# sjulier/Refactored_ORB_SLAM2

Hardware: AMD Instinct MI355X
Metric: frames/s (extract+match) at KITTI 1241×376, 2000 feat; 1/2/4/8 GPU + CPU ref (higher is better)
Workload: dtype u8; 1 GPU; kitti_stereo_1241x376_2000feat_8lvl: 2x ORBextractor + ComputeStereoMatches + SearchByProjection(cur,last); parallelism=frame-shard x1, collective=none, driver=torch, queries=one pass: orbfe_track_queries_stereo_device

## Files before the change

refactored_orb_slam2_amd/csrc/extract_kernels.hip:

```cpp
#include <stdlib.h>
#include <string.h>

#include "orbfe_internal.h"
#include "../../include/orb_pattern_data.h"

#define WAVE 64

__device__ __forceinline__ int wave_incl_scan(int v) {
  v += __builtin_amdgcn_update_dpp(0, v, 0x111, 0xf, 0xf, false);
  v += __builtin_amdgcn_update_dpp(0, v, 0x112, 0xf, 0xf, false);
  v += __builtin_amdgcn_update_dpp(0, v, 0x114, 0xf, 0xf, false);
  v += __builtin_amdgcn_update_dpp(0, v, 0x118, 0xf, 0xf, false);
  v += __builtin_amdgcn_update_dpp(0, v, 0x142, 0xa, 0xf, false);
  v += __builtin_amdgcn_update_dpp(0, v, 0x143, 0xc, 0xf, false);
  return v;
}

template <int T>
__device__ __forceinline__ int block_incl_scan_t(int v, int* tmp, int* total) {
  const int tid = threadIdx.x;
  const int lane = tid & (WAVE - 1), wid = tid >> 6;
  int s = wave_incl_scan(v);
  if (T == WAVE) {
    *total = __builtin_amdgcn_readlane(s, WAVE - 1);
// ... 377 lines not shown
#if FC_TIMING
__device__ unsigned long long g_fc_prof[4096 * 8];
#define FC_T(i) do { const uint32_t _t = (uint32_t)__builtin_readcyclecounter(); tacc##i += _t - tprev; tprev = _t; } while (0)
extern "C" int orbfe_debug_fc_profile(unsigned long long* out, int reset) {
  static unsigned long long h[4096 * 8];
  if (hipMemcpyFromSymbol(h, HIP_SYMBOL(g_fc_prof), sizeof(h)) != hipSuccess) return 1;
  for (int i = 0; i < 8; i++) out[i] = 0;
  for (int sl = 0; sl < 4096; sl++)
    for (int i = 0; i < 8; i++) out[i] += h[sl * 8 + i];
  if (reset) { memset(h, 0, sizeof(h)); if (hipMemcpyToSymbol(HIP_SYMBOL(g_fc_prof), h, sizeof(h)) != hipSuccess) return 1; }
  return 0;
}
#else
#define FC_T(i)
#endif
#ifndef FC_SCALAR_CELL
#define FC_SCALAR_CELL 1
#endif
#ifndef FC_PE_COND
#define FC_PE_COND 1
#endif
#ifndef FC_WAVES_PER_EU
#define FC_WAVES_PER_EU 7
#endif
#ifndef FC_WG_WAVES
#define FC_WG_WAVES 4
#endif
__host__ __device__ inline int fc_wave_lds(int rows_max, int pb, int sc_bytes, int nbw) {
  return rows_max * pb + sc_bytes + nbw * 4 + FC_LIST_CAP * 2 + (FC_T2_QUEUE ? FC_Q1_CAP * 2 : 0) + FC_LDS_PAD;
}
template <int PB, int NLD>
__global__ __launch_bounds__(64 * FC_WG_WAVES, FC_WAVES_PER_EU) void fast_cells_kernel(PyrView pyr, const CellDesc* __restrict__ cells,
                                                          const FastGroup* __restrict__ runs, int n_runs, int total_cells,
                                                          int rows_max, int sc_bytes, int nbw, int32_t* __restrict__ cell_cnt,
                                                          uint32_t* __restrict__ slots, unsigned long long slots_per_image,
                                                          int ini_th, int min_th, int xcd_run_shift) {
  extern __shared__ __attribute__((aligned(16))) uint8_t fc_smem[];
  const int lane = threadIdx.x & (WAVE - 1), wid = __builtin_amdgcn_readfirstlane((int)(threadIdx.x >> 6));
  uint8_t* tile = fc_smem + wid * fc_wave_lds(rows_max, PB, sc_bytes, nbw);
  uint8_t* sc = tile + rows_max * PB;
  uint32_t* scb = reinterpret_cast<uint32_t*>(sc + sc_bytes);
  uint16_t* list = reinterpret_cast<uint16_t*>(scb + nbw);
#if FC_T2_QUEUE
  uint16_t* q1 = list + FC_LIST_CAP;
#endif
  int img = blockIdx.y;
  const int nblk = (n_runs + FC_WG_WAVES - 1) / FC_WG_WAVES;
  const int q = blockIdx.x >> 3;
  const int unit = 8 << (xcd_run_shift < 0 ? 0 : xcd_run_shift);
  int bid = (xcd_run_shift < 0 || (int)blockIdx.x >= (nblk / unit) * unit)
                ? (int)blockIdx.x
                : ((q >> xcd_run_shift) << (xcd_run_shift + 3)) + ((blockIdx.x & 7) << xcd_run_shift) +
                      (q & ((1 << xcd_run_shift) - 1));
  if (xcd_run_shift == -2) {
    const unsigned gx = gridDim.x;
    const unsigned lin = blockIdx.y * gx + blockIdx.x;
    const unsigned grp = lin / (8u * gx);
    if (8u * grp + 8u <= gridDim.y) {
      const unsigned within = lin - grp * 8u * gx;
      img = (int)(8u * grp + (within & 7u));
      bid = (int)(within >> 3);
    }
  }
  const int rid = bid * FC_WG_WAVES + wid;
  if (rid >= n_runs) return;
  const FastGroup g = runs[rid];
  const int level = g.level;
  const int pitch = pyr.pitch[level];
  const uint8_t* plane = pyr.base[level] + (size_t)img * pyr.img_stride[level];
  const uint32_t tile_a = (uint32_t)(uintptr_t)tile;

#if FC_TIMING
  uint32_t tacc0 = 0, tacc1 = 0, tacc2 = 0, tacc3 = 0, tacc4 = 0, tacc5 = 0, tprev = (uint32_t)__builtin_readcyclecounter();
#endif
  static_assert(sizeof(CellDesc) == 32, "eight dwords");
  auto load_cell = [&](int idx) {
    const __attribute__((address_space(4))) uint32_t* q =
        (const __attribute__((address_space(4))) uint32_t*)(uintptr_t)(cells + __builtin_amdgcn_readfirstlane(idx));
    CellDesc c;
    uint32_t w[8];
#pragma unroll
    for (int j = 0; j < 8; j++) w[j] = q[j];
    __builtin_memcpy(&c, w, sizeof(c));
    return c;
  };
  for (int k = 0; k < g.n_cells; k++) {
    const CellDesc cd = FC_SCALAR_CELL ? load_cell(g.first_cell + k) : cells[g.first_cell + k];
    uint4 pv[NLD];
    uint32_t pe[NLD];
    {
      const int ndq = ((cd.x0 & 15) + (((cd.x0 & 15) + 3) & 1) + cd.cols + 15) >> 4;
      const uint8_t* src = plane + (size_t)cd.y0 * pitch + (cd.x0 & ~15);
      const bool ltiled = (pyr.tiled >> level) & 1u;
      const uint32_t tstep = (uint32_t)(pitch >> 4) << 7;
      auto chunk_ptr = [&](int r, int c) {
        const int y = cd.y0 + r;
        return ltiled ? plane + (uint32_t)(y >> 3) * tstep + ((uint32_t)(((cd.x0 & ~15) >> 4) + c) << 7) + (uint32_t)((y & 7) * 16)
                      : src + (size_t)r * pitch + 16 * c;
      };
      auto front_ptr = [&](int r, int c, const uint8_t* p) {
        return ltiled ? p - 128 + 12 : p - 4;
      };
      if constexpr (PB == 64) {
        const int c = min(lane & 3, ndq - 1);
#pragma unroll
        for (int kk = 0; kk < NLD; kk++) {
          const int r = min((lane >> 2) + 16 * kk, cd.rows - 1);
          const uint8_t* p = chunk_ptr(r, c);          pv[kk] = *reinterpret_cast<const uint4*>(p);
#if FC_PE_COND
          pe[kk] = ((cd.x0 & 15) + 3) & 1 ? *reinterpret_cast<const uint32_t*>(front_ptr(r, c, p)) : 0u;
#else
          pe[kk] = *reinterpret_cast<const uint32_t*>(front_ptr(r, c, p));
#endif
        }
      } else {
        const int items = cd.rows * ndq;
        const float inv = 1.0f / (float)ndq;
#pragma unroll
        for (int kk = 0; kk < NLD; kk++) {
          const int i = min(lane + WAVE * kk, items - 1);
          const int r = (int)((i + 0.5f) * inv), c = i - r * ndq;
          const uint8_t* p = chunk_ptr(r, c);
          pv[kk] = *reinterpret_cast<const uint4*>(p);
          pe[kk] = *reinterpret_cast<const uint32_t*>(front_ptr(r, c, p));
        }
      }
    }
#if FC_TIMING
    asm volatile("s_waitcnt vmcnt(0)" ::: "memory");
    FC_T(0);
#endif
    const int cols = cd.cols, rows = cd.rows;
    const int xo = cd.x0 & 15, sh = (xo + 3) & 1, xs = xo + sh;
    const int ndq = (xs + cols + 15) >> 4;
    const int th = rows - 6, tw = cols - 6;
    const int c_lo = xs + 3, c_hi = xs + cols - 3;
    const int SCP = tw + 2;
    const int bsh = tw > 32 ? 6 : 5;
    {
      const int items = rows * ndq;
      const float inv = 1.0f / (float)ndq;
#pragma unroll
      for (int kk = 0; kk < NLD; kk++) {
        int r, c;
        if constexpr (PB == 64) { r = min((lane >> 2) + 16 * kk, rows - 1); c = min(lane & 3, ndq - 1); }
        else { const int i = min(lane + WAVE * kk, items - 1); r = (int)((i + 0.5f) * inv); c = i - r * ndq; }
        uint4 d = pv[kk];
        if (sh) {
          d.w = __builtin_amdgcn_alignbyte(d.w, d.z, 3);
          d.z = __builtin_amdgcn_alignbyte(d.z, d.y, 3);
          d.y = __builtin_amdgcn_alignbyte(d.y, d.x, 3);
          d.x = __builtin_amdgcn_alignbyte(d.x, pe[kk], 3);
        }
        *reinterpret_cast<uint4*>(tile + r * PB + 16 * c) = d;
      }
      const int nsc = ((th + 2) * SCP + 15) >> 4;
      for (int i = lane; i < nsc; i += WAVE) reinterpret_cast<uint4*>(sc)[i] = make_uint4(0, 0, 0, 0);
    }
    FC_T(1);

    auto score_list = [&](int n, bool mark, int th_cur) {
      int n_end = n;
      for (int done = 0; done < n_end;) {
        const int start = done;
        const int lim = min(start + WAVE, n_end);
        const int i = start + lane;
        done = lim;
        uint32_t en = i < lim ? list[i] : 0u;
        int e = (int)(en & 0x3fffu);
        int y = PB == 64 ? (e >> 6) : (int)((e + 0.5f) * (1.0f / PB));
        int x = e - y * PB;
// ... 44 lines not shown
            atomicOr(&scb[p >> 5], 1u << (p & 31));
          }
        }
      }
    };

    uint32_t keep[2] = {0u, 0u};
    int total = 0;
    bool was_flushed = false;
    for (int pass = 0; pass < 2; pass++) {
      const int th_cur = pass ? min_th : ini_th;
      const uint32_t C = (uint32_t)(0x8000 - th_cur - 1) * 0x00010001u;
      bool flushed = false;
      int wcnt = 0;
      if (th > 0 && tw > 0) {
        const int ppr = cd.ppr;
        const int RI = cd.ri;
        const int rl = (int)((lane + 0.5f) * cd.inv_ppr), pl = lane - rl * ppr;
        const bool lane_ok = rl < RI;
        const int n_it = cd.n_it;
        const int x = c_lo + 2 * pl;
        const bool odd2 = (x & 2) != 0;
        const uint32_t selV = odd2 ? 0x0c030c02u : 0x0c010c00u;
#if !FC_T2_QUEUE
        const uint32_t selX = odd2 ? 0x0c010c00u : 0x0c030c02u;
#endif
        const uint32_t selM = odd2 ? 0x0c040c03u : 0x0c020c01u;
        const uint32_t selP = odd2 ? 0x0c020c01u : 0x0c040c03u;
        uint32_t a0 = tile_a + rl * PB + ((x >> 2) << 2) - 4;
        uint32_t a1 = a0 + (odd2 ? 4u : 0u);
#if !(FC_T2_QUEUE && FC_T1_ASM)
        const uint32_t ec = (uint32_t)(3 * PB + 4 + (x & 3)) - tile_a;
        int rows_left = lane_ok ? th - rl : 0;
#endif
#if FC_T2_QUEUE && FC_T1_ASM
        const unsigned long long m_full = __ballot(lane_ok), m_last = __ballot(lane_ok && rl < th - (n_it - 1) * RI);
        const uint32_t oddbit = odd2 ? 1u : 0u;
        const uint32_t q_base = (uint32_t)(uintptr_t)q1, q_limit = q_base + 2u * WAVE;
        uint32_t q_addr = q_base;
        int it = 0;
        for (int phase = 0; phase < 2; phase++) {
          const unsigned long long actm = phase ? m_last : m_full;
          const int nit = __builtin_amdgcn_readfirstlane(phase ? n_it : n_it - 1);
          const int step = __builtin_amdgcn_readfirstlane(RI * PB);
          for (;;) {
            if (it < nit) {
              uint32_t tV, tA, tB, tC, tD, tE;
              uint32_t sc_;
              asm volatile(
                  "1:\n\t"
                  "ds_read2_b32 v[64:65], %[a0] offset0:1 offset1:%[K61]\n\t"
                  "ds_read2_b32 v[66:67], %[a0] offset0:%[K30] offset1:%[K31]\n\t"
                  "ds_read2_b32 v[68:69], %[a1] offset0:%[K31] offset1:%[K32]\n\t"
                  "s_add_u32 %[it], %[it], 1\n\t"
                  "s_waitcnt lgkmcnt(0)\n\t"
                  "v_perm_b32 %[tV], 0, v67, %[selV]\n\t"
                  "v_perm_b32 %[tA], 0, v64, %[selV]\n\t"
                  "v_perm_b32 %[tB], 0, v65, %[selV]\n\t"
                  "v_perm_b32 %[tC], v67, v66, %[selM]\n\t"
// ... 111 lines not shown
            const uint32_t D0 = (uint32_t)(pc >> 32), Dm = (uint32_t)pc;
            const uint32_t V = __builtin_amdgcn_perm(0u, D0, selV);
            const uint32_t Q8 = __builtin_amdgcn_perm(0u, (uint32_t)p08, selV), Q0 = __builtin_amdgcn_perm(0u, (uint32_t)(p08 >> 32), selV);
            const uint32_t Q12 = __builtin_amdgcn_perm(D0, Dm, selM);
            const uint32_t Q4 = __builtin_amdgcn_perm((uint32_t)(pp >> 32), (uint32_t)pp, selP);
            const uint32_t AD = V + C, AB = C - V;
            const uint32_t lo = pkmax(pkmin(Q0, Q8), pkmin(Q4, Q12));
            const uint32_t hi = pkmin(pkmax(Q0, Q8), pkmax(Q4, Q12));
            const uint32_t t1 = ((AD - lo) | (hi + AB)) & 0x80008000u;
            const unsigned long long m1 = __builtin_amdgcn_uicmp(t1, 0u, 33 ) & actm;
            if (m1 != 0ull) {
              const int r = __builtin_amdgcn_mbcnt_hi((uint32_t)(m1 >> 32), __builtin_amdgcn_mbcnt_lo((uint32_t)m1, (uint32_t)q1t));
              if ((t1 != 0u) & (rows_left > 0)) q1[r & (FC_Q1_CAP - 1)] = (uint16_t)(a0 + ec);
              q1t += __popcll(m1);
            }
            a0 += RI * PB; a1 += RI * PB; rows_left -= RI;
          }
          const int qn = q1t - q1h;
          if (it < n_it ? qn < WAVE : qn == 0) continue;
          const bool on = lane < qn;
          uint32_t e2 = q1[(q1h + lane) & (FC_Q1_CAP - 1)];
          e2 = on ? e2 : (uint32_t)(3 * PB + 4);
          q1h += qn < WAVE ? qn : WAVE;
          const uint32_t xx = PB == 64 ? (e2 & 63u) : e2 - (uint32_t)((int)((e2 + 0.5f) * (1.0f / PB))) * (uint32_t)PB;
          const uint32_t o2 = xx & 2u, k2 = o2 * 0x00010001u;
          const uint32_t sV = 0x0c010c00u + k2, sX = 0x0c030c02u - k2, sM = 0x0c020c01u + k2, sP = 0x0c040c03u - k2;
          const uint32_t b0 = tile_a + e2 - (uint32_t)(3 * PB + 4) - (xx & 3u);
          const uint32_t b1 = b0 + 2u * o2;
          unsigned long long p08, pc, pp, p62, p1014;
          asm volatile(
              "ds_read2_b32 %0, %5 offset0:1 offset1:%7\n\t"
// ... 27 lines not shown
            if (has0) list[i0] = (uint16_t)((G & 0xC000u) | e2);
            if (has1) list[i1] = (uint16_t)(((G >> 16) & 0xC000u) | (e2 + 1));
            wcnt += __popcll(m0) + __popcll(m1);
          }
          if (wcnt > FC_LIST_CAP - 2 * WAVE) {
            FC_T(2);
            if (!flushed)
              for (int i = lane; i < nbw; i += WAVE) scb[i] = 0;
            flushed = true;
            score_list(wcnt, true, th_cur);
            FC_T(3);
            wcnt = 0;
          }
        }
#else
        for (int it = 0; it < n_it; it++, a0 += RI * PB, a1 += RI * PB, rows_left -= RI) {
          const unsigned long long actm = __builtin_amdgcn_sicmp(rows_left, 0, 38 );
          const bool act = rows_left > 0;
          unsigned long long p08, pc, pp, p62, p1014;
          asm volatile(
              "ds_read2_b32 %0, %5 offset0:1 offset1:%7\n\t"
              "ds_read2_b32 %1, %5 offset0:%8 offset1:%9\n\t"
              "ds_read2_b32 %2, %6 offset0:%9 offset1:%10\n\t"
              "ds_read2_b32 %3, %6 offset0:%11 offset1:%12\n\t"
              "ds_read2_b32 %4, %6 offset0:%13 offset1:%14\n\t"
              "s_waitcnt lgkmcnt(2)"
              : "=&v"(p08), "=&v"(pc), "=&v"(pp), "=&v"(p62), "=&v"(p1014)
              : "v"(a0), "v"(a1), "n"(6 * PB / 4 + 1), "n"(3 * PB / 4), "n"(3 * PB / 4 + 1), "n"(3 * PB / 4 + 2),
                "n"(PB / 4 + 1), "n"(5 * PB / 4 + 1), "n"(PB / 4), "n"(5 * PB / 4)
              : "memory");
          const uint32_t D0 = (uint32_t)(pc >> 32), Dm = (uint32_t)pc;
// ... 28 lines not shown
            if (!flushed)
              for (int i = lane; i < nbw; i += WAVE) scb[i] = 0;
            flushed = true;
            score_list(wcnt, true, th_cur);
            FC_T(3);
            wcnt = 0;
          }
        }
#endif
        FC_T(2);
        score_list(wcnt, flushed, th_cur);
        FC_T(3);
      }

      if (!flushed) {
        uint32_t* slot = slots + (size_t)img * slots_per_image + cd.slot_off;
        int emitted = 0;
        for (int base = 0; base < wcnt; base += WAVE) {
          const int i = min(base + lane, wcnt - 1);
          const uint32_t en = list[i];
          const int e = (int)(en & 0x3fffu);
          const int y = PB == 64 ? (e >> 6) : (int)((e + 0.5f) * (1.0f / PB));
          const int x = e - y * PB;
          const int ty = y - 3, tx = x - c_lo;
          const uint8_t* s = sc + (ty + 1) * SCP + min(tx, tw - 1) + 1;
          const int v = s[0];
          const int n0 = s[-SCP - 1], n1 = s[-SCP], n2 = s[-SCP + 1], n3 = s[-1], n4 = s[1], n5 = s[SCP - 1], n6 = s[SCP], n7 = s[SCP + 1];
          const bool kp = (base + lane < wcnt) & (x < c_hi) & (v > n0) & (v > n1) & (v > n2) & (v > n3) & (v > n4) & (v > n5) & (v > n6) & (v > n7);
          const unsigned long long mk = __ballot(kp);
          const int off = __builtin_amdgcn_mbcnt_hi((uint32_t)(mk >> 32), __builtin_amdgcn_mbcnt_lo((uint32_t)mk, (uint32_t)emitted));
          const uint32_t rx = (uint32_t)(tx + 3 + cd.x0 - ORBFE_EDGE), ry = (uint32_t)(ty + 3 + cd.y0 - ORBFE_EDGE);
          if (kp && off < cd.slot_cap) slot[off] = rx | (ry << 12) | ((uint32_t)v << 24);
          emitted += __popcll(mk);
        }
        total = emitted;
      } else {
#pragma unroll
        for (int h = 0; h < 2; h++) {
          const int w = lane + WAVE * h;
          uint32_t m = w < nbw ? scb[w] : 0u;
          keep[h] = 0;
          while (m) {
            const int b = __ffs((int)m) - 1;
            m &= m - 1;
            const int p = w * 32 + b;
            const int ty = p >> bsh, tx = p & ((1 << bsh) - 1);
            const uint8_t* s = sc + (ty + 1) * SCP + tx + 1;
// ... 3 lines not shown
            if (kp) keep[h] |= 1u << b;
          }
        }
        total = __popcll(__ballot(keep[0] != 0u || keep[1] != 0u));
      }
      was_flushed = flushed;
      FC_T(4);
      if (total != 0 || pass == 1) break;
      {
        const int nsc = ((th + 2) * SCP + 15) >> 4;
        for (int i = lane; i < nsc; i += WAVE) reinterpret_cast<uint4*>(sc)[i] = make_uint4(0, 0, 0, 0);
      }
    }

    if (!was_flushed) {
      if (lane == 0) cell_cnt[(size_t)img * total_cells + g.first_cell + k] = total < cd.slot_cap ? total : cd.slot_cap;
      FC_T(5);
    } else {
      const int pk = __popc(keep[0]) | (__popc(keep[1]) << 16);
      const int in = wave_incl_scan(pk);
      const int tot = __builtin_amdgcn_readlane(in, WAVE - 1);
      const int tot0 = tot & 0xffff, n_out = tot0 + (tot >> 16);
      const int ex = in - pk;
      uint32_t* slot = slots + (size_t)img * slots_per_image + cd.slot_off;
#pragma unroll
      for (int h = 0; h < 2; h++) {
        int off = h ? tot0 + (ex >> 16) : (ex & 0xffff);
        uint32_t mask = keep[h];
        const int w = lane + WAVE * h;
        while (mask) {
          const int b = __ffs((int)mask) - 1;
          mask &= mask - 1;
          const int p = w * 32 + b;
          const int ty = p >> bsh, tx = p & ((1 << bsh) - 1);
          const uint32_t sv = sc[(ty + 1) * SCP + tx + 1];
          const uint32_t rx = (uint32_t)(tx + 3 + cd.x0 - ORBFE_EDGE), ry = (uint32_t)(ty + 3 + cd.y0 - ORBFE_EDGE);
          if (off < cd.slot_cap) slot[off] = rx | (ry << 12) | (sv << 24);
          off++;
        }
      }
      if (lane == 0) cell_cnt[(size_t)img * total_cells + g.first_cell + k] = n_out < cd.slot_cap ? n_out : cd.slot_cap;
      FC_T(5);
    }
  }
#if FC_TIMING
  if (lane == 0) {
    unsigned long long* pr = g_fc_prof + (size_t)((rid * 2654435761u) >> 20) * 8;
    atomicAdd(&pr[0], (unsigned long long)tacc0); atomicAdd(&pr[1], (unsigned long long)tacc1);
    atomicAdd(&pr[2], (unsigned long long)tacc2); atomicAdd(&pr[3], (unsigned long long)tacc3);
    atomicAdd(&pr[4], (unsigned long long)tacc4); atomicAdd(&pr[5], (unsigned long long)tacc5);
    atomicAdd(&pr[6], 1ull);
    atomicAdd(&pr[7], (unsigned long long)g.n_cells);
  }
#endif
}

// ... 1559 lines not shown
    if (mode == 3)
      hipLaunchKernelGGL((pyr_resize_dot_kernel<32, 42, 336>), dim3(nb), block, 0, s, src, spitch, (unsigned long long)simg, dst,
                         dpitch, (unsigned long long)dimg, dw, dh, xt, yt, tiles_x, tiles_y, n_tiles);
    else
      hipLaunchKernelGGL((pyr_resize_dot_kernel<32, 42, RS_COLS>), dim3(nb), block, 0, s, src, spitch, (unsigned long long)simg, dst,
                         dpitch, (unsigned long long)dimg, dw, dh, xt, yt, tiles_x, tiles_y, n_tiles);
  }
  else if (mode >= 1)
    hipLaunchKernelGGL(pyr_resize_lds16_kernel, dim3((dw + 255) / 256, (dh + 15) / 16, n_images), block, 0, s, src, spitch,
                       (unsigned long long)simg, dst, dpitch, (unsigned long long)dimg, dw, dh, xt, yt);
  else
    hipLaunchKernelGGL(pyr_resize_kernel, grid, block, 0, s, src, spitch, (unsigned long long)simg, dst, dpitch,
                       (unsigned long long)dimg, dw, dh, xt, yt);
}

void orbfe_launch_fast_cells(const PyrView& pyr, const CellDesc* cells, const FastGroup* groups, int n_groups, int total_cells,
                             int cell_rows, int cell_span, int sc_max, int bits_max, int32_t* cell_cnt, uint32_t* slots,
                             unsigned long long slots_per_image, int ini_th, int min_th, int n_images, hipStream_t s) {
  if (n_groups == 0) return;
  const int run_shift = -2;
  const int pb = cell_span <= 64 ? 64 : 96;
  const int sc_bytes = (sc_max + 15) & ~15;
  const int nbw = bits_max <= 64 * 32 ? 64 : 128;
  const size_t lds = (size_t)FC_WG_WAVES * fc_wave_lds(cell_rows, pb, sc_bytes, nbw);
  const bool small = cell_rows <= 48;
  dim3 grid4((n_groups + FC_WG_WAVES - 1) / FC_WG_WAVES, n_images);
#define FC_LAUNCH(PBV, NLDV)                                                                                                   \
  hipLaunchKernelGGL((fast_cells_kernel<PBV, NLDV>), grid4, dim3(64 * FC_WG_WAVES), lds, s, pyr, cells, groups, n_groups, total_cells,       \
                     cell_rows, sc_bytes, nbw, cell_cnt, slots, slots_per_image, ini_th, min_th, run_shift)
  if (lds > 48 * 1024) {
    (void)hipFuncSetAttribute(reinterpret_cast<const void*>(fast_cells_kernel<96, 7>), hipFuncAttributeMaxDynamicSharedMemorySize, (int)lds);
    (void)hipFuncSetAttribute(reinterpret_cast<const void*>(fast_cells_kernel<64, 7>), hipFuncAttributeMaxDynamicSharedMemorySize, (int)lds);
  }
  if (pb == 64 && small) FC_LAUNCH(64, 3);
  else if (pb == 64) FC_LAUNCH(64, 7);
  else FC_LAUNCH(96, 7);
#undef FC_LAUNCH
}

void orbfe_launch_octree(const OctParams& p, int n_images, size_t lds_bytes, hipStream_t s) {
  dim3 block(ORBFE_OCT_THREADS), grid(n_images, p.n_levels);
  hipLaunchKernelGGL(octree_select_kernel, grid, block, lds_bytes, s, p);
}
// ... 80 lines not shown
```

refactored_orb_slam2_amd/csrc/extractor.cpp:

```cpp
#include <math.h>
#include <stdarg.h>
#include <stdio.h>
#include <stdlib.h>
#include <string.h>

#include <algorithm>
#include <atomic>
#include <mutex>
#include <vector>

#include "orbfe_internal.h"

void orbfe_launch_copy0(const uint8_t* src, int sstride, size_t simg, uint8_t* dst, int dpitch, size_t dimg, int w,
                        int h, int n_images, int tiled, hipStream_t s);
int orbfe_set_octree_lds(size_t lds_bytes);
int orbfe_upload_pattern_floats();

static thread_local char g_err[512] = "";
void orbfe_set_error(const char* fmt, ...) {
  va_list ap;
  va_start(ap, fmt);
  vsnprintf(g_err, sizeof(g_err), fmt, ap);
  va_end(ap);
}
// ... 210 lines not shown
    const LevelGeom& g = e->lg[l];
    fits = fits && g.w >= 8 && g.h >= 8;
    const int nch = (g.w + 12 + ORBFE_BLUR_CHUNK - 1) / ORBFE_BLUR_CHUNK;
    for (int c = 0; c < nch; c++) e->strips.push_back(BlurStrip{(int16_t)l, (int16_t)c});
    e->blur_b_off[l] = (uint32_t)e->blur_tab.size();
    e->blur_tab.resize(e->blur_tab.size() + (size_t)nch * 3 * 1024);
    int8_t* bt = reinterpret_cast<int8_t*>(e->blur_tab.data() + e->blur_b_off[l]);
    for (int c = 0; c < nch; c++)
      for (int gg = 0; gg < 3; gg++)
        for (int lane = 0; lane < 64; lane++)
          for (int j = 0; j < 16; j++)
            put(bt[(((size_t)c * 3 + gg) * 64 + lane) * 16 + j],
                blur_coef(ORBFE_BLUR_CHUNK * c - 16 + 16 * (lane >> 4) + j, ORBFE_BLUR_CHUNK * c - 12 + 16 * gg + (lane & 15), g.w));
  }
  return fits;
}


static int build_plan(orbfe_extractor* e, int w, int h) {
  if (e->plan_w == w && e->plan_h == h) return ORBFE_OK;
  if (w < 1 || h < 1 || w > 4095 || h > 4095) {
    orbfe_set_error("unsupported image size %dx%d (1..4095)", w, h);
    return ORBFE_ERR_INVALID;
  }
  const int nl = e->prm.n_levels;
  e->plan_w = e->plan_h = 0;
  size_t off = 0;
  for (int l = 0; l < nl; l++) {
    LevelGeom& g = e->lg[l];
    g.w = cv_round_f((float)w * e->inv_scale[l]);
// ... 60 lines not shown
          e->fc_rows = std::max(e->fc_rows, (int)c.rows);
          e->fc_span = std::max(e->fc_span, (c.x0 & 15) + 1 + (int)c.cols);
          e->fc_sc = std::max(e->fc_sc, (th + 2) * (tw + 2));
          e->fc_bits = std::max(e->fc_bits, th * (tw > 32 ? 64 : 32));
          c.slot_off = (uint32_t)slot_off;
          slot_off += cap;
          level_slots += cap;
          e->cells.push_back(c);
        }
        const int n_row = (int)(e->cells.size() - row_first);
        const int G = std::max(1, std::min(ORBFE_FG_MAX, (ORBFE_FG_MAX_WIDTH - 6) / wCell));
        const int n_grp = (n_row + G - 1) / G;
        int done = 0;
        for (int k = 0; k < n_grp; k++) {
          const int cnt = (n_row - done + (n_grp - k) - 1) / (n_grp - k);
          const CellDesc& a = e->cells[row_first + done];
          const CellDesc& b = e->cells[row_first + done + cnt - 1];
          FastGroup fg;
          fg.first_cell = (int32_t)(row_first + done);
          fg.n_cells = (int16_t)cnt; fg.level = (int16_t)l;
          fg.x0 = a.x0; fg.y0 = a.y0; fg.width = (int16_t)(b.x0 + b.cols - a.x0); fg.rows = a.rows;
          fg.wcell = (int16_t)wCell; fg.pad = 0;
          e->groups.push_back(fg);
          done += cnt;
        }
      }
      const int nIni = (int)roundf(width / height);
      if (nIni < 1 || nIni > ORBFE_MAX_INI) {
        orbfe_set_error("level %d aspect ratio gives nIni=%d (supported 1..%d)", l, nIni, ORBFE_MAX_INI);
        return ORBFE_ERR_INVALID;
      }
      o.n_ini = nIni;
      o.hX = width / nIni;
    }
    o.n_cells = (int)e->cells.size() - o.cell_begin;
    o.kp_cap = std::max(o.N + 3, 4 * o.n_ini) + 1;
    o.kp_off = kp_off;
    kp_off += o.kp_cap;
    maxM = std::max(maxM, o.kp_cap);
    o.key_off = key_off;
    o.key_cap = (int)std::min<size_t>(level_slots, 0xFFFFFF);
    key_off += level_slots;
  }
  for (CellDesc& c : e->cells) {
    const int tw = std::max(c.cols - 6, 0), th = std::max(c.rows - 6, 0);
    const int ppr = std::max((tw + 1) >> 1, 1), ri = std::max(64 / ppr, 1);
    c.ppr = (int16_t)ppr; c.ri = (int16_t)ri; c.n_it = (int16_t)((th + ri - 1) / ri);
    c.inv_ppr = 1.0f / (float)ppr;
  }
  std::vector<ResizeTap> hxt[ORBFE_MAX_LEVELS], hyt[ORBFE_MAX_LEVELS];
  for (int l = 1; l < nl; l++) {
    std::vector<ResizeTap>&xt = hxt[l], &yt = hyt[l];
    build_taps(e->lg[l - 1].w, e->lg[l].w, true, xt);
    build_taps(e->lg[l - 1].h, e->lg[l].h, false, yt);
    bool ok = true;
    for (int x0 = 0; x0 < (int)xt.size() && ok; x0 += 256) {
      const int xl = std::min<int>(x0 + 255, (int)xt.size() - 1);
      const int sxa = xt[x0].s0 & ~15;
      if ((((xt[xl].s1 - sxa) >> 4) + 1) * 16 > 560) ok = false;
    }
    for (int y0 = 0; y0 < (int)yt.size() && ok; y0 += 16) {
      const int yl = std::min<int>(y0 + 15, (int)yt.size() - 1);
      if (yt[yl].s1 - yt[y0].s0 + 1 > 34) ok = false;
    }
// ... 86 lines not shown
      return ORBFE_ERR_INVALID;
    }
    if (e->oct_lds > 64 * 1024) {
      int rc = orbfe_set_octree_lds(e->oct_lds);
      if (rc != 0) {
        orbfe_set_error("hipFuncSetAttribute(max dynamic LDS %zu) failed: %d", e->oct_lds, rc);
        return ORBFE_ERR_HIP;
      }
    }
  }
  int rc;
  if ((rc = upload(e->d_cells, e->cells.data(), e->cells.size() * sizeof(CellDesc), e->stream))) return rc;
  if ((rc = upload(e->d_groups, e->groups.data(), e->groups.size() * sizeof(FastGroup), e->stream))) return rc;
  {
    std::vector<FastGroup> g1(e->cells.size());
    for (size_t i = 0; i < e->cells.size(); i++) {
      memset(&g1[i], 0, sizeof(FastGroup));
      g1[i].first_cell = (int32_t)i;
      g1[i].n_cells = 1;
      g1[i].level = e->cells[i].level;
    }
    if ((rc = upload(e->d_groups1, g1.data(), g1.size() * sizeof(FastGroup), e->stream))) return rc;
    HIPCHK(hipStreamSynchronize(e->stream));
  }
  if ((rc = upload(e->d_tiles, e->tiles.data(), e->tiles.size() * sizeof(BlurTile), e->stream))) return rc;
  if ((rc = upload(e->d_strips, e->strips.data(), e->strips.size() * sizeof(BlurStrip), e->stream))) return rc;
  if ((rc = upload(e->d_blur_tab, e->blur_tab.data(), e->blur_tab.size(), e->stream))) return rc;
  for (int l = 1; l < nl; l++) {
    if ((rc = upload(e->d_xt[l], hxt[l].data(), hxt[l].size() * sizeof(ResizeTap), e->stream))) return rc;
    if ((rc = upload(e->d_yt[l], hyt[l].data(), hyt[l].size() * sizeof(ResizeTap), e->stream))) return rc;
  }
  HIPCHK(hipStreamSynchronize(e->stream));
  e->plan_w = w;
  e->plan_h = h;
  e->cap_images = 0;
  return ORBFE_OK;
// ... 167 lines not shown
        rz.dimg = e->lg[l + 1].plane;
        rz.dpitch = pv.pitch[l + 1]; rz.dw = pv.w[l + 1]; rz.dh = pv.h[l + 1];
        rz.dst_tiled = (int)((pv.tiled >> (l + 1)) & 1u);
        rz.xt = (const ResizeTap*)e->d_xt[l + 1].p;
        rz.yt = (const ResizeTap*)e->d_yt[l + 1].p;
        orbfe_launch_blur_level(pv, bv, lt, e->tile_count[l], &rz, n_images, s);
      } else {
        if (l + 1 < nl) resize_step(l + 1);
        orbfe_launch_blur_level(pv, bv, lt, e->tile_count[l], nullptr, n_images, s);
      }
    }
  }
  {
    StageTimer t(e, s, ORBFE_STAGE_FAST);
    const bool few = n_images <= 8;
    orbfe_launch_fast_cells(pv, (const CellDesc*)e->d_cells.p, (const FastGroup*)(few ? e->d_groups1.p : e->d_groups.p),
                            few ? e->total_cells : (int)e->groups.size(), e->total_cells, e->fc_rows, e->fc_span, e->fc_sc,
                            e->fc_bits, (int32_t*)e->d_cell_cnt.p, (uint32_t*)e->d_slots.p, e->slots_per_image,
                            e->prm.ini_th_fast, e->prm.min_th_fast, n_images, s);
  }
  {
    StageTimer t(e, s, ORBFE_STAGE_OCTREE);
    OctParams op;
    memset(&op, 0, sizeof(op));
    for (int l = 0; l < nl; l++) op.lv[l] = e->oct[l];
    op.cells = (const CellDesc*)e->d_cells.p;
    op.cell_cnt = (const int32_t*)e->d_cell_cnt.p;
    op.slots = (const uint32_t*)e->d_slots.p;
    op.cell_off = (int32_t*)e->d_cell_off.p;
    op.gkeys = (unsigned long long*)e->d_gkeys.p;
    op.lvl_kp = (uint32_t*)e->d_lvl_kp.p;
// ... 581 lines not shown
```

refactored_orb_slam2_amd/csrc/orbfe_internal.h:

```cpp
#pragma once
#include <hip/hip_runtime.h>
#include <stdint.h>

#include "../../include/orbfe.h"

#define ORBFE_EDGE 16
#define ORBFE_CELL_MAX 66
#ifndef ORBFE_BLUR_TILE_H
#define ORBFE_BLUR_TILE_H 56
#endif
#define ORBFE_MAX_INI 256
#ifndef ORBFE_OCT_THREADS
#define ORBFE_OCT_THREADS 256
#endif

struct PyrView {
  const uint8_t* base[ORBFE_MAX_LEVELS];
  unsigned long long img_stride[ORBFE_MAX_LEVELS];
  int pitch[ORBFE_MAX_LEVELS];
  int w[ORBFE_MAX_LEVELS], h[ORBFE_MAX_LEVELS];
  int n_levels;
  unsigned tiled;
};

// ... 19 lines not shown
  int16_t shift_x, shift_y;
  int16_t slot_cap;
  uint32_t slot_off;
  int16_t ppr, ri, n_it, pad;
  float inv_ppr;
};

#ifndef ORBFE_FG_MAX
#define ORBFE_FG_MAX 4
#define ORBFE_FG_MAX_WIDTH 176
#endif
struct FastGroup {
  int32_t first_cell;
  int16_t n_cells, level;
  int16_t x0, y0, width, rows;
  int16_t wcell, pad;
};

struct OctLevel {
  int cell_begin, n_cells;
  int N;
  int n_ini;
  float hX;
  int width, height;
  int kp_off, kp_cap;
  unsigned long long key_off;
  int key_cap;
  int ff_depth;
};

struct OctParams {
  OctLevel lv[ORBFE_MAX_LEVELS];
// ... 50 lines not shown
#define ORBFE_BLUR_WINDOW 32
struct BlurStrip {
  int16_t level, chunk;
};
struct BlurMfmaParams {
  const BlurStrip* strips;
  int n_strips;
  const uint8_t* tab;
  uint32_t b_off[ORBFE_MAX_LEVELS];
  uint32_t t_off;
  int use;
};

void orbfe_launch_resize(const uint8_t* src, int spitch, size_t simg, uint8_t* dst, int dpitch, size_t dimg, int dw,
                         int dh, const ResizeTap* xt, const ResizeTap* yt, int n_images, int mode, hipStream_t s);
void orbfe_launch_fast_cells(const PyrView& pyr, const CellDesc* cells, const FastGroup* groups, int n_groups, int total_cells,
                             int cell_rows, int cell_span, int sc_max, int bits_max, int32_t* cell_cnt, uint32_t* slots,
                             unsigned long long slots_per_image, int ini_th, int min_th, int n_images, hipStream_t s);
void orbfe_launch_octree(const OctParams& p, int n_images, size_t lds_bytes, hipStream_t s);
void orbfe_launch_blur(const PyrView& src, const PyrView& dst, const BlurTile* tiles, int n_tiles, const BlurMfmaParams& mf,
                       int n_images, hipStream_t s);
void orbfe_launch_blur_level(const PyrView& src, const PyrView& dst, const BlurTile* tiles, int n_tiles, const LevelResize* rz,
                             int n_images, hipStream_t s);
void orbfe_launch_describe(const DescribeParams& p, int n_images, hipStream_t s);
size_t orbfe_octree_lds_bytes(int max_nodes, int lds_keys);
```

Measured before the change: 113,500 frames/s.

## Fold per-cell descriptors into 64-byte run records and hoist per-cell address math

Per-cell descriptor fields (cols, slot cap/offset, ppr/ri/n_it layout) move into an enlarged 64-byte FastGroup run record, loaded once per wave via scalar loads, so the FAST kernel no longer reads a CellDesc per cell. Row offsets, slot and count pointers and layout parameters are hoisted out of the per-cell loop, and cell x0 is advanced by a fixed stride. Host code validates that every run is uniform and rejects configurations that do not fit. This cuts scalar memory traffic and per-cell integer work, at the cost of a stricter layout assumption and more live registers.

```diff
diff --git a/refactored_orb_slam2_amd/csrc/extract_kernels.hip b/refactored_orb_slam2_amd/csrc/extract_kernels.hip
--- a/refactored_orb_slam2_amd/csrc/extract_kernels.hip
+++ b/refactored_orb_slam2_amd/csrc/extract_kernels.hip
@@ -415,8 +415,8 @@
 #else
 #define FC_T(i)
 #endif
-#ifndef FC_SCALAR_CELL
-#define FC_SCALAR_CELL 1
+#ifndef FC_BOUND
+#define FC_BOUND 0
 #endif
 #ifndef FC_PE_COND
 #define FC_PE_COND 1
@@ -431,13 +431,14 @@
   return rows_max * pb + sc_bytes + nbw * 4 + FC_LIST_CAP * 2 + (FC_T2_QUEUE ? FC_Q1_CAP * 2 : 0) + FC_LDS_PAD;
 }
 template <int PB, int NLD>
-__global__ __launch_bounds__(64 * FC_WG_WAVES, FC_WAVES_PER_EU) void fast_cells_kernel(PyrView pyr, const CellDesc* __restrict__ cells,
+__global__ __launch_bounds__(64 * FC_WG_WAVES, FC_WAVES_PER_EU) void fast_cells_kernel(PyrView pyr,
                                                           const FastGroup* __restrict__ runs, int n_runs, int total_cells,
                                                           int rows_max, int sc_bytes, int nbw, int32_t* __restrict__ cell_cnt,
                                                           uint32_t* __restrict__ slots, unsigned long long slots_per_image,
                                                           int ini_th, int min_th, int xcd_run_shift) {
   extern __shared__ __attribute__((aligned(16))) uint8_t fc_smem[];
-  const int lane = threadIdx.x & (WAVE - 1), wid = __builtin_amdgcn_readfirstlane((int)(threadIdx.x >> 6));
+  int lane = threadIdx.x & (WAVE - 1);
+  const int wid = __builtin_amdgcn_readfirstlane((int)(threadIdx.x >> 6));
   uint8_t* tile = fc_smem + wid * fc_wave_lds(rows_max, PB, sc_bytes, nbw);
   uint8_t* sc = tile + rows_max * PB;
   uint32_t* scb = reinterpret_cast<uint32_t*>(sc + sc_bytes);
@@ -465,7 +466,16 @@
   }
   const int rid = bid * FC_WG_WAVES + wid;
   if (rid >= n_runs) return;
-  const FastGroup g = runs[rid];
+  static_assert(sizeof(FastGroup) == 64, "sixteen dwords");
+  FastGroup g;
+  {
+    const __attribute__((address_space(4))) uint32_t* q =
+        (const __attribute__((address_space(4))) uint32_t*)(uintptr_t)(runs + __builtin_amdgcn_readfirstlane(rid));
+    uint32_t w[16];
+#pragma unroll
+    for (int j = 0; j < 16; j++) w[j] = q[j];
+    __builtin_memcpy(&g, w, sizeof(g));
+  }
   const int level = g.level;
   const int pitch = pyr.pitch[level];
   const uint8_t* plane = pyr.base[level] + (size_t)img * pyr.img_stride[level];
@@ -474,78 +484,129 @@
 #if FC_TIMING
   uint32_t tacc0 = 0, tacc1 = 0, tacc2 = 0, tacc3 = 0, tacc4 = 0, tacc5 = 0, tprev = (uint32_t)__builtin_readcyclecounter();
 #endif
-  static_assert(sizeof(CellDesc) == 32, "eight dwords");
-  auto load_cell = [&](int idx) {
-    const __attribute__((address_space(4))) uint32_t* q =
-        (const __attribute__((address_space(4))) uint32_t*)(uintptr_t)(cells + __builtin_amdgcn_readfirstlane(idx));
-    CellDesc c;
-    uint32_t w[8];
-#pragma unroll
-    for (int j = 0; j < 8; j++) w[j] = q[j];
-    __builtin_memcpy(&c, w, sizeof(c));
-    return c;
+  const int y0 = g.y0, rows = g.rows, th = rows - 6;
+  const bool ltiled = (pyr.tiled >> level) & 1u;
+  const uint32_t tstep = (uint32_t)(pitch >> 4) << 7;
+  const uint32_t cstride = ltiled ? 128u : 16u;
+  const uint8_t* plane_front = plane - (ltiled ? 116 : 4);
+  auto row_off = [&](int r) {
+    const uint32_t y = (uint32_t)(y0 + r);
+    return ltiled ? (y >> 3) * tstep + (y & 7u) * 16u : y * (uint32_t)pitch;
   };
-  for (int k = 0; k < g.n_cells; k++) {
-    const CellDesc cd = FC_SCALAR_CELL ? load_cell(g.first_cell + k) : cells[g.first_cell + k];
+  constexpr bool HOIST_ROWS = PB == 64 && NLD <= 3;
+  uint32_t g_row[HOIST_ROWS ? NLD : 1], l_row[HOIST_ROWS ? NLD : 1];
+  if constexpr (HOIST_ROWS) {
+#pragma unroll
+    for (int kk = 0; kk < NLD; kk++) {
+      const int r = min((lane >> 2) + 16 * kk, rows - 1);
+      g_row[kk] = row_off(r);
+      l_row[kk] = (uint32_t)(r * PB);
+    }
+  }
+  const int lane3 = lane & 3;
+  uint32_t* slot = slots + (size_t)img * slots_per_image + g.slot_off;
+  int32_t* cnt = cell_cnt + (size_t)img * total_cells + g.first_cell;
+  int cols, tw, SCP, bsh, nsc, slot_cap, n_it, step;
+  [[maybe_unused]] unsigned long long m_full, m_last;
+#if !(FC_T2_QUEUE && FC_T1_ASM)
+  int RI_c, rows_left0;
+#endif
+  uint32_t a_row, pl2;
+  auto set_layout = [&](int cols_, int cap_, int ppr, int RI, int n_it_, float inv_ppr) {
+    cols = cols_; slot_cap = cap_; n_it = n_it_;
+    tw = cols_ - 6; SCP = tw + 2;
+    bsh = tw > 32 ? 6 : 5;
+    nsc = ((th + 2) * SCP + 15) >> 4;
+    const int rl = (int)((lane + 0.5f) * inv_ppr), pl = lane - rl * ppr;
+    const bool lane_ok = rl < RI;
+    m_full = __ballot(lane_ok); m_last = __ballot(lane_ok && rl < th - (n_it_ - 1) * RI);
+    step = __builtin_amdgcn_readfirstlane(RI * PB);
+    a_row = tile_a + (uint32_t)(rl * PB) - 4u;
+    pl2 = (uint32_t)(2 * pl);
+#if !(FC_T2_QUEUE && FC_T1_ASM)
+    RI_c = RI; rows_left0 = lane_ok ? th - rl : 0;
+#endif
+  };
+  constexpr bool LAYOUT_PER_RUN = PB == 64;
+  if constexpr (LAYOUT_PER_RUN) set_layout(g.cols, g.slot_cap, g.ppr, g.ri, g.n_it, g.inv_ppr);
+#if FC_T2_QUEUE
+  [[maybe_unused]] const uint32_t q_base = (uint32_t)(uintptr_t)q1, q_limit = q_base + 2u * WAVE;
+#endif
+  int x0 = g.x0;
+  int k_other = g.last_differs ? g.n_cells - 1 : -1;
+  asm volatile("" : "+s"(k_other));
+  int sh = 0, c_lo = 0, c_hi = 0, vc = 0;
+  for (int k = 0; k < g.n_cells; k++, x0 += g.wcell, slot += g.slot_cap, cnt++) {
+    if constexpr (PB == 96) asm volatile("" : "+v"(lane));
+    if (!LAYOUT_PER_RUN || k == k_other) {
+      const bool o = k == k_other;
+      int ppr_l = __builtin_amdgcn_readfirstlane(o ? g.ppr_last : g.ppr), ri_l = __builtin_amdgcn_readfirstlane(o ? g.ri_last : g.ri);
+      int inv_l = __builtin_amdgcn_readfirstlane(__builtin_bit_cast(int, o ? g.inv_ppr_last : g.inv_ppr));
+      asm volatile("" : "+s"(ppr_l), "+s"(ri_l), "+s"(inv_l));
+      set_layout(o ? g.cols_last : g.cols, o ? g.slot_cap_last : g.slot_cap, ppr_l, ri_l, o ? g.n_it_last : g.n_it,
+                 __builtin_bit_cast(float, inv_l));
+    }
+    int chunk0 = x0 >> 4;
+#if FC_BOUND
+    if (k > 0 && cols == g.cols) {
+      chunk0 = max(min(chunk0, (pitch >> 4) - PB / 16), 1);
+    } else
+#endif
+    {
+      const int xo = x0 & 15;
+      sh = (xo + 3) & 1;
+      const int xs = xo + sh;
+      const int ndq = (xs + cols + 15) >> 4;
+      c_lo = xs + 3; c_hi = xs + cols - 3;
+      if constexpr (PB == 64) vc = min(lane3, ndq - 1);
+      else vc = ndq;
+    }
     uint4 pv[NLD];
     uint32_t pe[NLD];
-    {
-      const int ndq = ((cd.x0 & 15) + (((cd.x0 & 15) + 3) & 1) + cd.cols + 15) >> 4;
-      const uint8_t* src = plane + (size_t)cd.y0 * pitch + (cd.x0 & ~15);
-      const bool ltiled = (pyr.tiled >> level) & 1u;
-      const uint32_t tstep = (uint32_t)(pitch >> 4) << 7;
-      auto chunk_ptr = [&](int r, int c) {
-        const int y = cd.y0 + r;
-        return ltiled ? plane + (uint32_t)(y >> 3) * tstep + ((uint32_t)(((cd.x0 & ~15) >> 4) + c) << 7) + (uint32_t)((y & 7) * 16)
-                      : src + (size_t)r * pitch + 16 * c;
-      };
-      auto front_ptr = [&](int r, int c, const uint8_t* p) {
-        return ltiled ? p - 128 + 12 : p - 4;
-      };
-      if constexpr (PB == 64) {
-        const int c = min(lane & 3, ndq - 1);
-#pragma unroll
-        for (int kk = 0; kk < NLD; kk++) {
-          const int r = min((lane >> 2) + 16 * kk, cd.rows - 1);
-          const uint8_t* p = chunk_ptr(r, c);          pv[kk] = *reinterpret_cast<const uint4*>(p);
+    int lane_c = lane;
+    if constexpr (!HOIST_ROWS) asm volatile("" : "+v"(lane_c));
+    if constexpr (PB == 64) {
+      const uint32_t coff = (uint32_t)(chunk0 + vc) * cstride;
+#pragma unroll
+      for (int kk = 0; kk < NLD; kk++) {
+        uint32_t off = coff;
+        if constexpr (HOIST_ROWS) off += g_row[kk];
+        else off += row_off(min((lane_c >> 2) + 16 * kk, rows - 1));
+        pv[kk] = *reinterpret_cast<const uint4*>(plane + off);
 #if FC_PE_COND
-          pe[kk] = ((cd.x0 & 15) + 3) & 1 ? *reinterpret_cast<const uint32_t*>(front_ptr(r, c, p)) : 0u;
+        pe[kk] = sh ? *reinterpret_cast<const uint32_t*>(plane_front + off) : 0u;
 #else
-          pe[kk] = *reinterpret_cast<const uint32_t*>(front_ptr(r, c, p));
-#endif
-        }
-      } else {
-        const int items = cd.rows * ndq;
-        const float inv = 1.0f / (float)ndq;
-#pragma unroll
-        for (int kk = 0; kk < NLD; kk++) {
-          const int i = min(lane + WAVE * kk, items - 1);
-          const int r = (int)((i + 0.5f) * inv), c = i - r * ndq;
-          const uint8_t* p = chunk_ptr(r, c);
-          pv[kk] = *reinterpret_cast<const uint4*>(p);
-          pe[kk] = *reinterpret_cast<const uint32_t*>(front_ptr(r, c, p));
-        }
+        pe[kk] = *reinterpret_cast<const uint32_t*>(plane_front + off);
+#endif
+      }
+    } else {
+      const int ndq = vc;
+      const int items = rows * ndq;
+      const float inv = 1.0f / (float)ndq;
+#pragma unroll
+      for (int kk = 0; kk < NLD; kk++) {
+        const int i = min(lane_c + WAVE * kk, items - 1);
+        const int r = (int)((i + 0.5f) * inv), c = i - r * ndq;
+        const uint32_t off = row_off(r) + (uint32_t)(chunk0 + c) * cstride;
+        pv[kk] = *reinterpret_cast<const uint4*>(plane + off);
+        pe[kk] = *reinterpret_cast<const uint32_t*>(plane_front + off);
       }
     }
 #if FC_TIMING
     asm volatile("s_waitcnt vmcnt(0)" ::: "memory");
     FC_T(0);
 #endif
-    const int cols = cd.cols, rows = cd.rows;
-    const int xo = cd.x0 & 15, sh = (xo + 3) & 1, xs = xo + sh;
-    const int ndq = (xs + cols + 15) >> 4;
-    const int th = rows - 6, tw = cols - 6;
-    const int c_lo = xs + 3, c_hi = xs + cols - 3;
-    const int SCP = tw + 2;
-    const int bsh = tw > 32 ? 6 : 5;
     {
-      const int items = rows * ndq;
-      const float inv = 1.0f / (float)ndq;
 #pragma unroll
       for (int kk = 0; kk < NLD; kk++) {
-        int r, c;
-        if constexpr (PB == 64) { r = min((lane >> 2) + 16 * kk, rows - 1); c = min(lane & 3, ndq - 1); }
-        else { const int i = min(lane + WAVE * kk, items - 1); r = (int)((i + 0.5f) * inv); c = i - r * ndq; }
+        uint32_t st;
+        if constexpr (HOIST_ROWS) st = l_row[kk] + 16u * (uint32_t)vc;
+        else if constexpr (PB == 64) st = (uint32_t)(min((lane_c >> 2) + 16 * kk, rows - 1) * PB + 16 * vc);
+        else {
+          const int ndq = vc, i = min(lane_c + WAVE * kk, rows * ndq - 1);
+          const int r = (int)((i + 0.5f) * (1.0f / (float)ndq));
+          st = (uint32_t)(r * PB + 16 * (i - r * ndq));
+        }
         uint4 d = pv[kk];
         if (sh) {
           d.w = __builtin_amdgcn_alignbyte(d.w, d.z, 3);
@@ -553,9 +614,8 @@
           d.y = __builtin_amdgcn_alignbyte(d.y, d.x, 3);
           d.x = __builtin_amdgcn_alignbyte(d.x, pe[kk], 3);
         }
-        *reinterpret_cast<uint4*>(tile + r * PB + 16 * c) = d;
-      }
-      const int nsc = ((th + 2) * SCP + 15) >> 4;
+        *reinterpret_cast<uint4*>(tile + st) = d;
+      }
       for (int i = lane; i < nsc; i += WAVE) reinterpret_cast<uint4*>(sc)[i] = make_uint4(0, 0, 0, 0);
     }
     FC_T(1);
@@ -630,35 +690,26 @@
       bool flushed = false;
       int wcnt = 0;
       if (th > 0 && tw > 0) {
-        const int ppr = cd.ppr;
-        const int RI = cd.ri;
-        const int rl = (int)((lane + 0.5f) * cd.inv_ppr), pl = lane - rl * ppr;
-        const bool lane_ok = rl < RI;
-        const int n_it = cd.n_it;
-        const int x = c_lo + 2 * pl;
-        const bool odd2 = (x & 2) != 0;
-        const uint32_t selV = odd2 ? 0x0c030c02u : 0x0c010c00u;
+        const uint32_t x = (uint32_t)c_lo + pl2;
+        const uint32_t oddbit = (x >> 1) & 1u, k2 = oddbit * 0x00020002u;
+        const uint32_t selV = 0x0c010c00u + k2;
 #if !FC_T2_QUEUE
-        const uint32_t selX = odd2 ? 0x0c010c00u : 0x0c030c02u;
-#endif
-        const uint32_t selM = odd2 ? 0x0c040c03u : 0x0c020c01u;
-        const uint32_t selP = odd2 ? 0x0c020c01u : 0x0c040c03u;
-        uint32_t a0 = tile_a + rl * PB + ((x >> 2) << 2) - 4;
-        uint32_t a1 = a0 + (odd2 ? 4u : 0u);
+        const uint32_t selX = 0x0c030c02u - k2;
+#endif
+        const uint32_t selM = 0x0c020c01u + k2;
+        const uint32_t selP = 0x0c040c03u - k2;
+        uint32_t a0 = a_row + (x & ~3u);
+        uint32_t a1 = a0 + 4u * oddbit;
 #if !(FC_T2_QUEUE && FC_T1_ASM)
         const uint32_t ec = (uint32_t)(3 * PB + 4 + (x & 3)) - tile_a;
-        int rows_left = lane_ok ? th - rl : 0;
+        int rows_left = rows_left0;
 #endif
 #if FC_T2_QUEUE && FC_T1_ASM
-        const unsigned long long m_full = __ballot(lane_ok), m_last = __ballot(lane_ok && rl < th - (n_it - 1) * RI);
-        const uint32_t oddbit = odd2 ? 1u : 0u;
-        const uint32_t q_base = (uint32_t)(uintptr_t)q1, q_limit = q_base + 2u * WAVE;
         uint32_t q_addr = q_base;
         int it = 0;
         for (int phase = 0; phase < 2; phase++) {
           const unsigned long long actm = phase ? m_last : m_full;
-          const int nit = __builtin_amdgcn_readfirstlane(phase ? n_it : n_it - 1);
-          const int step = __builtin_amdgcn_readfirstlane(RI * PB);
+          const int nit = phase ? n_it : n_it - 1;
           for (;;) {
             if (it < nit) {
               uint32_t tV, tA, tB, tC, tD, tE;
@@ -800,7 +851,7 @@
               if ((t1 != 0u) & (rows_left > 0)) q1[r & (FC_Q1_CAP - 1)] = (uint16_t)(a0 + ec);
               q1t += __popcll(m1);
             }
-            a0 += RI * PB; a1 += RI * PB; rows_left -= RI;
+            a0 += step; a1 += step; rows_left -= RI_c;
           }
           const int qn = q1t - q1h;
           if (it < n_it ? qn < WAVE : qn == 0) continue;
@@ -858,7 +909,7 @@
           }
         }
 #else
-        for (int it = 0; it < n_it; it++, a0 += RI * PB, a1 += RI * PB, rows_left -= RI) {
+        for (int it = 0; it < n_it; it++, a0 += step, a1 += step, rows_left -= RI_c) {
           const unsigned long long actm = __builtin_amdgcn_sicmp(rows_left, 0, 38 );
           const bool act = rows_left > 0;
           unsigned long long p08, pc, pp, p62, p1014;
@@ -917,7 +968,6 @@
       }
 
       if (!flushed) {
-        uint32_t* slot = slots + (size_t)img * slots_per_image + cd.slot_off;
         int emitted = 0;
         for (int base = 0; base < wcnt; base += WAVE) {
           const int i = min(base + lane, wcnt - 1);
@@ -932,8 +982,8 @@
           const bool kp = (base + lane < wcnt) & (x < c_hi) & (v > n0) & (v > n1) & (v > n2) & (v > n3) & (v > n4) & (v > n5) & (v > n6) & (v > n7);
           const unsigned long long mk = __ballot(kp);
           const int off = __builtin_amdgcn_mbcnt_hi((uint32_t)(mk >> 32), __builtin_amdgcn_mbcnt_lo((uint32_t)mk, (uint32_t)emitted));
-          const uint32_t rx = (uint32_t)(tx + 3 + cd.x0 - ORBFE_EDGE), ry = (uint32_t)(ty + 3 + cd.y0 - ORBFE_EDGE);
-          if (kp && off < cd.slot_cap) slot[off] = rx | (ry << 12) | ((uint32_t)v << 24);
+          const uint32_t rx = (uint32_t)(tx + 3 + x0 - ORBFE_EDGE), ry = (uint32_t)(ty + 3 + y0 - ORBFE_EDGE);
+          if (kp && off < slot_cap) slot[off] = rx | (ry << 12) | ((uint32_t)v << 24);
           emitted += __popcll(mk);
         }
         total = emitted;
@@ -967,7 +1017,7 @@
     }
 
     if (!was_flushed) {
-      if (lane == 0) cell_cnt[(size_t)img * total_cells + g.first_cell + k] = total < cd.slot_cap ? total : cd.slot_cap;
+      if (lane == 0) *cnt = total < slot_cap ? total : slot_cap;
       FC_T(5);
     } else {
       const int pk = __popc(keep[0]) | (__popc(keep[1]) << 16);
@@ -975,7 +1025,6 @@
       const int tot = __builtin_amdgcn_readlane(in, WAVE - 1);
       const int tot0 = tot & 0xffff, n_out = tot0 + (tot >> 16);
       const int ex = in - pk;
-      uint32_t* slot = slots + (size_t)img * slots_per_image + cd.slot_off;
 #pragma unroll
       for (int h = 0; h < 2; h++) {
         int off = h ? tot0 + (ex >> 16) : (ex & 0xffff);
@@ -987,12 +1036,12 @@
           const int p = w * 32 + b;
           const int ty = p >> bsh, tx = p & ((1 << bsh) - 1);
           const uint32_t sv = sc[(ty + 1) * SCP + tx + 1];
-          const uint32_t rx = (uint32_t)(tx + 3 + cd.x0 - ORBFE_EDGE), ry = (uint32_t)(ty + 3 + cd.y0 - ORBFE_EDGE);
-          if (off < cd.slot_cap) slot[off] = rx | (ry << 12) | (sv << 24);
+          const uint32_t rx = (uint32_t)(tx + 3 + x0 - ORBFE_EDGE), ry = (uint32_t)(ty + 3 + y0 - ORBFE_EDGE);
+          if (off < slot_cap) slot[off] = rx | (ry << 12) | (sv << 24);
           off++;
         }
       }
-      if (lane == 0) cell_cnt[(size_t)img * total_cells + g.first_cell + k] = n_out < cd.slot_cap ? n_out : cd.slot_cap;
+      if (lane == 0) *cnt = n_out < slot_cap ? n_out : slot_cap;
       FC_T(5);
     }
   }
@@ -2582,7 +2631,7 @@
                        (unsigned long long)dimg, dw, dh, xt, yt);
 }
 
-void orbfe_launch_fast_cells(const PyrView& pyr, const CellDesc* cells, const FastGroup* groups, int n_groups, int total_cells,
+void orbfe_launch_fast_cells(const PyrView& pyr, const FastGroup* groups, int n_groups, int total_cells,
                              int cell_rows, int cell_span, int sc_max, int bits_max, int32_t* cell_cnt, uint32_t* slots,
                              unsigned long long slots_per_image, int ini_th, int min_th, int n_images, hipStream_t s) {
   if (n_groups == 0) return;
@@ -2594,7 +2643,7 @@
   const bool small = cell_rows <= 48;
   dim3 grid4((n_groups + FC_WG_WAVES - 1) / FC_WG_WAVES, n_images);
 #define FC_LAUNCH(PBV, NLDV)                                                                                                   \
-  hipLaunchKernelGGL((fast_cells_kernel<PBV, NLDV>), grid4, dim3(64 * FC_WG_WAVES), lds, s, pyr, cells, groups, n_groups, total_cells,       \
+  hipLaunchKernelGGL((fast_cells_kernel<PBV, NLDV>), grid4, dim3(64 * FC_WG_WAVES), lds, s, pyr, groups, n_groups, total_cells,       \
                      cell_rows, sc_bytes, nbw, cell_cnt, slots, slots_per_image, ini_th, min_th, run_shift)
   if (lds > 48 * 1024) {
     (void)hipFuncSetAttribute(reinterpret_cast<const void*>(fast_cells_kernel<96, 7>), hipFuncAttributeMaxDynamicSharedMemorySize, (int)lds);
diff --git a/refactored_orb_slam2_amd/csrc/extractor.cpp b/refactored_orb_slam2_amd/csrc/extractor.cpp
--- a/refactored_orb_slam2_amd/csrc/extractor.cpp
+++ b/refactored_orb_slam2_amd/csrc/extractor.cpp
@@ -248,6 +248,31 @@
                 blur_coef(ORBFE_BLUR_CHUNK * c - 16 + 16 * (lane >> 4) + j, ORBFE_BLUR_CHUNK * c - 12 + 16 * gg + (lane & 15), g.w));
   }
   return fits;
+}
+
+bool orbfe_fill_run(const CellDesc* cells, int first, int n, int wcell, FastGroup* g) {
+  if (n < 1 || n > ORBFE_FG_MAX) return false;
+  const CellDesc& a = cells[first];
+  const CellDesc& b = cells[first + n - 1];
+  for (int k = 0; k < n; k++) {
+    const CellDesc& c = cells[first + k];
+    if (c.level != a.level || c.y0 != a.y0 || c.rows != a.rows) return false;
+    if (c.x0 != a.x0 + k * wcell || c.x0 < ORBFE_EDGE) return false;
+    if (c.slot_off != a.slot_off + (uint32_t)k * (uint32_t)a.slot_cap) return false;
+    if (k < n - 1 && (c.cols != a.cols || c.slot_cap != a.slot_cap)) return false;
+    if (k < n - 1 && (c.ppr != a.ppr || c.ri != a.ri || c.n_it != a.n_it || c.inv_ppr != a.inv_ppr)) return false;
+  }
+  memset(g, 0, sizeof(*g));
+  g->first_cell = first;
+  g->n_cells = (int16_t)n; g->level = a.level;
+  g->x0 = a.x0; g->y0 = a.y0; g->width = (int16_t)(b.x0 + b.cols - a.x0); g->rows = a.rows;
+  g->wcell = (int16_t)wcell;
+  g->cols = a.cols; g->cols_last = b.cols; g->last_differs = b.cols != a.cols;
+  g->slot_cap = a.slot_cap; g->slot_cap_last = b.slot_cap;
+  g->slot_off = a.slot_off;
+  g->ppr = a.ppr; g->ri = a.ri; g->n_it = a.n_it; g->inv_ppr = a.inv_ppr;
+  g->ppr_last = b.ppr; g->ri_last = b.ri; g->n_it_last = b.n_it; g->inv_ppr_last = b.inv_ppr;
+  return true;
 }
 
 
@@ -338,13 +363,11 @@
         int done = 0;
         for (int k = 0; k < n_grp; k++) {
           const int cnt = (n_row - done + (n_grp - k) - 1) / (n_grp - k);
-          const CellDesc& a = e->cells[row_first + done];
-          const CellDesc& b = e->cells[row_first + done + cnt - 1];
           FastGroup fg;
+          memset(&fg, 0, sizeof(fg));
           fg.first_cell = (int32_t)(row_first + done);
-          fg.n_cells = (int16_t)cnt; fg.level = (int16_t)l;
-          fg.x0 = a.x0; fg.y0 = a.y0; fg.width = (int16_t)(b.x0 + b.cols - a.x0); fg.rows = a.rows;
-          fg.wcell = (int16_t)wCell; fg.pad = 0;
+          fg.n_cells = (int16_t)cnt;
+          fg.wcell = (int16_t)wCell;
           e->groups.push_back(fg);
           done += cnt;
         }
@@ -372,6 +395,12 @@
     c.ppr = (int16_t)ppr; c.ri = (int16_t)ri; c.n_it = (int16_t)((th + ri - 1) / ri);
     c.inv_ppr = 1.0f / (float)ppr;
   }
+  for (FastGroup& fg : e->groups)
+    if (!orbfe_fill_run(e->cells.data(), fg.first_cell, fg.n_cells, fg.wcell, &fg)) {
+      orbfe_set_error("FAST cells %d..%d are not one run (level, y0, rows, x step, slots or widths differ)", (int)fg.first_cell,
+                      (int)(fg.first_cell + fg.n_cells - 1));
+      return ORBFE_ERR_INVALID;
+    }
   std::vector<ResizeTap> hxt[ORBFE_MAX_LEVELS], hyt[ORBFE_MAX_LEVELS];
   for (int l = 1; l < nl; l++) {
     std::vector<ResizeTap>&xt = hxt[l], &yt = hyt[l];
@@ -488,12 +517,11 @@
   if ((rc = upload(e->d_groups, e->groups.data(), e->groups.size() * sizeof(FastGroup), e->stream))) return rc;
   {
     std::vector<FastGroup> g1(e->cells.size());
-    for (size_t i = 0; i < e->cells.size(); i++) {
-      memset(&g1[i], 0, sizeof(FastGroup));
-      g1[i].first_cell = (int32_t)i;
-      g1[i].n_cells = 1;
-      g1[i].level = e->cells[i].level;
-    }
+    for (size_t i = 0; i < e->cells.size(); i++)
+      if (!orbfe_fill_run(e->cells.data(), (int)i, 1, 0, &g1[i])) {
+        orbfe_set_error("FAST cell %d does not fit a run record", (int)i);
+        return ORBFE_ERR_INVALID;
+      }
     if ((rc = upload(e->d_groups1, g1.data(), g1.size() * sizeof(FastGroup), e->stream))) return rc;
     HIPCHK(hipStreamSynchronize(e->stream));
   }
@@ -691,7 +719,7 @@
   {
     StageTimer t(e, s, ORBFE_STAGE_FAST);
     const bool few = n_images <= 8;
-    orbfe_launch_fast_cells(pv, (const CellDesc*)e->d_cells.p, (const FastGroup*)(few ? e->d_groups1.p : e->d_groups.p),
+    orbfe_launch_fast_cells(pv, (const FastGroup*)(few ? e->d_groups1.p : e->d_groups.p),
                             few ? e->total_cells : (int)e->groups.size(), e->total_cells, e->fc_rows, e->fc_span, e->fc_sc,
                             e->fc_bits, (int32_t*)e->d_cell_cnt.p, (uint32_t*)e->d_slots.p, e->slots_per_image,
                             e->prm.ini_th_fast, e->prm.min_th_fast, n_images, s);
diff --git a/refactored_orb_slam2_amd/csrc/orbfe_internal.h b/refactored_orb_slam2_amd/csrc/orbfe_internal.h
--- a/refactored_orb_slam2_amd/csrc/orbfe_internal.h
+++ b/refactored_orb_slam2_amd/csrc/orbfe_internal.h
@@ -57,8 +57,18 @@
   int32_t first_cell;
   int16_t n_cells, level;
   int16_t x0, y0, width, rows;
-  int16_t wcell, pad;
+  int16_t wcell, cols;
+  int16_t cols_last, last_differs;
+  int16_t slot_cap, slot_cap_last;
+  uint32_t slot_off;
+  int16_t ppr, ri, n_it, pad0;
+  float inv_ppr;
+  int16_t ppr_last, ri_last, n_it_last, pad1;
+  float inv_ppr_last;
+  uint32_t pad2[2];
 };
+static_assert(sizeof(FastGroup) == 64, "fast_cells_kernel loads sixteen dwords");
+bool orbfe_fill_run(const CellDesc* cells, int first, int n, int wcell, FastGroup* g);
 
 struct OctLevel {
   int cell_begin, n_cells;
@@ -139,7 +149,7 @@
 
 void orbfe_launch_resize(const uint8_t* src, int spitch, size_t simg, uint8_t* dst, int dpitch, size_t dimg, int dw,
                          int dh, const ResizeTap* xt, const ResizeTap* yt, int n_images, int mode, hipStream_t s);
-void orbfe_launch_fast_cells(const PyrView& pyr, const CellDesc* cells, const FastGroup* groups, int n_groups, int total_cells,
+void orbfe_launch_fast_cells(const PyrView& pyr, const FastGroup* groups, int n_groups, int total_cells,
                              int cell_rows, int cell_span, int sc_max, int bits_max, int32_t* cell_cnt, uint32_t* slots,
                              unsigned long long slots_per_image, int ini_th, int min_th, int n_images, hipStream_t s);
 void orbfe_launch_octree(const OctParams& p, int n_images, size_t lds_bytes, hipStream_t s);
```

New measurement: 114,600 frames/s (median of 6 runs). Within noise of the previous version (+1.0%).
